# zeehu/generative_ranking_recommender

Measured on AMD Instinct MI355X. Metric: vectors quantized/sec (3-level RQ, 512-d), higher is better.
Workload: dtype f32

## Files before the change

### generative_ranking_recommender_amd/_lib.py

```python
from __future__ import annotations

import contextlib
import ctypes
import fcntl
import os
import subprocess
import tempfile
from pathlib import Path

PKG = Path(__file__).resolve().parent
REPO = PKG.parent
LIB_PATH = PKG / "librqsid.so"
SRCS = [PKG / "csrc" / "rqsid.hip", PKG / "csrc" / "assign.hip", PKG / "csrc" / "assign_stream.hip",
        PKG / "csrc" / "assign_resident.hip", PKG / "csrc" / "assign_rows.hip", PKG / "csrc" / "assign_pc.hip",
        PKG / "csrc" / "auction.hip",
        PKG / "csrc" / "auction_seg.hip", PKG / "csrc" / "quant_error.hip", PKG / "csrc" / "assign_topk.hip",
        PKG / "csrc" / "beam.hip", PKG / "csrc" / "silhouette.hip"]
DEPS = SRCS + [PKG / "csrc" / "internal.h", PKG / "csrc" / "assign_common.h", PKG / "csrc" / "assign_plan.h",
               PKG / "csrc" / "topk_kernel.h", PKG / "csrc" / "exact_row.h"]
HEADER = REPO / "include" / "rqsid.h"
IO_LIB_PATH = PKG / "librqsid_io.so"
IO_SRCS = [PKG / "csrc" / "csv_loader.cpp"]
IO_HEADER = REPO / "include" / "rqsid_io.h"
IO_FLAGS = ["-O3", "-std=c++17", "-Wall", "-shared", "-fPIC", "-pthread"]

HIPCC_FLAGS = ["--offload-arch=gfx950", "-O3", "-std=c++17", "-fno-slp-vectorize", "-shared", "-fPIC"]

c_i32, c_i64, c_f32, c_vp, c_char_p = ctypes.c_int32, ctypes.c_int64, ctypes.c_float, ctypes.c_void_p, ctypes.c_char_p

SIGNATURES = {
    "rqsid_version": (c_i32, []),
    "rqsid_last_error": (c_char_p, []),
    "rqsid_build_flags": (c_i32, []),
    "rqsid_prepare_centers": (c_i32, [c_vp, c_i64, c_i32, c_vp, c_vp, c_vp]),
    "rqsid_prepare_centers_hi": (c_i32, [c_vp, c_i64, c_i32, c_vp, c_vp]),
    "rqsid_bucket_workspace_bytes": (c_i64, [c_i64, c_i32]),
    "rqsid_bucket": (c_i32, [c_vp, c_i64, c_i32, c_i32, c_vp, c_vp, c_vp, c_vp, c_i64, c_vp]),
    "rqsid_assign_tile_rows": (c_i32, []),
    "rqsid_assign_workspace_bytes": (c_i64, [c_i64]),
    "rqsid_assign": (c_i32, [c_vp, c_i64, c_i32, c_vp, c_i32, c_vp, c_vp, c_i64,
                             c_vp, c_vp, c_vp, c_vp, c_i32,
                             c_vp, c_vp, c_i32, c_vp, c_vp, c_vp,
                             c_i32, c_i32, c_vp, c_vp, c_vp, c_vp, c_vp, c_vp,
                             c_vp, c_vp, c_i32, c_vp, c_i64, c_vp]),
    "rqsid_assign_x": (c_i32, [c_vp, c_i32, c_i64, c_i32, c_vp, c_i32, c_vp, c_vp, c_i64,
                               c_vp, c_vp, c_vp, c_vp, c_i32,
                               c_vp, c_vp, c_i32, c_vp, c_vp, c_vp,
                               c_i32, c_i32, c_vp, c_vp, c_vp, c_vp, c_vp, c_vp,
                               c_vp, c_vp, c_i32, c_vp, c_i64, c_vp]),
    "rqsid_pair_table_bytes": (c_i64, [c_i32]),
    "rqsid_pair_table": (c_i32, [c_vp, c_i32, c_vp, c_i32, c_i32, c_vp, c_vp, c_i32, c_vp, c_vp, c_vp]),
    "rqsid_assign_pair": (c_i32, [c_vp, c_i32, c_i64, c_i32, c_vp, c_i32, c_vp, c_vp, c_i64,
                                  c_vp, c_vp, c_vp, c_vp, c_i32,
                                  c_vp, c_vp, c_i32, c_vp, c_vp, c_vp,
                                  c_i32, c_i32, c_vp, c_vp, c_vp, c_vp, c_vp, c_vp,
                                  c_vp, c_vp, c_i32, c_vp, c_i64, c_vp, c_vp]),
    "rqsid_assign_plan_pair": (c_i32, [c_i32, c_i64, c_i32, c_i32, c_i32, c_i32, c_i32, c_i32, c_i32, c_i32, c_i32]),
    "rqsid_assign_topk_workspace_bytes": (c_i64, [c_i64, c_i32]),
    "rqsid_assign_topk": (c_i32, [c_vp, c_i32, c_i64, c_i32, c_vp, c_i32, c_vp, c_vp, c_i64,
                                  c_vp, c_vp, c_i32,
                                  c_vp, c_vp, c_i32, c_vp, c_vp, c_vp,
                                  c_i32, c_i32, c_vp, c_vp, c_vp, c_vp, c_vp, c_vp,
                                  c_i32, c_vp, c_vp, c_vp, c_vp, c_i64, c_vp]),
    "rqsid_beam_expand_workspace_bytes": (c_i64, [c_i64, c_i32]),
    "rqsid_beam_expand": (c_i32, [c_vp, c_i32, c_i64, c_i32, c_i32, c_vp, c_i32, c_vp, c_vp, c_i64,
                                  c_vp, c_vp, c_i32,
                                  c_vp, c_vp, c_i32, c_vp, c_vp, c_vp,
                                  c_i32, c_i32, c_vp, c_vp, c_vp, c_vp, c_vp, c_vp,
                                  c_i32, c_vp, c_vp, c_vp, c_vp, c_i64, c_vp]),
    "rqsid_beam_merge": (c_i32, [c_i64, c_i32, c_i32, c_i32, c_i32, c_vp, c_vp, c_vp, c_vp, c_vp, c_vp,
                                 c_i32, c_i32, c_i32, c_vp, c_vp, c_vp, c_vp, c_vp, c_vp, c_vp]),
    "rqsid_residual": (c_i32, [c_vp, c_i64, c_i32, c_vp, c_i32, c_vp, c_vp, c_i32, c_i32, c_vp, c_vp]),
    "rqsid_quant_error_workspace_bytes": (c_i64, [c_i64]),
    "rqsid_quant_error": (c_i32, [c_vp, c_i32, c_i64, c_i32, c_vp, c_i32, c_i32,
                                  c_vp, c_i32, c_vp, c_vp, c_i32, c_vp, c_vp, c_i32, c_vp,
                                  c_vp, c_vp, c_vp, c_vp, c_i64, c_vp]),
    "rqsid_silhouette_tile_rows": (c_i32, []),
    "rqsid_silhouette_workspace_bytes": (c_i64, [c_i64, c_i32, c_i32]),
    "rqsid_silhouette": (c_i32, [c_vp, c_i32, c_i64, c_i32, c_vp, c_i32, c_vp, c_vp, c_i32, c_vp, c_vp, c_i32,
                                 c_vp, c_vp, c_vp, c_vp, c_vp, c_i64, c_vp]),
    "rqsid_scale_groups": (c_i32, [c_vp, c_i64, c_i32, c_vp, c_i32, c_vp, c_vp, c_vp]),
    "rqsid_centroid_tile_rows": (c_i32, []),
    "rqsid_centroid_accumulate": (c_i32, [c_vp, c_i32, c_vp, c_i32, c_vp, c_vp, c_i64, c_vp, c_vp]),
    "rqsid_centroid_finalize": (c_i32, [c_vp, c_vp, c_i32, c_i32, c_vp, c_vp]),
    "rqsid_match_workspace_bytes": (c_i64, [c_i32]),
    "rqsid_match_to_candidates": (c_i32, [c_vp, c_i32, c_i32, c_vp, c_vp, c_vp, c_vp, c_vp, c_i64, c_vp]),
    "rqsid_pairwise_distance": (c_i32, [c_vp, c_i64, c_i32, c_vp, c_i32, c_vp, c_vp]),
    "rqsid_auction_scores": (c_i32, [c_vp, c_i64, c_i32, c_vp, c_i32, c_i32, c_vp, c_vp]),
    "rqsid_auction_workspace_bytes": (c_i64, [c_i64, c_i32]),
    "rqsid_auction_lap_half": (c_i32, [c_vp, c_i32, c_i64, c_i32, c_vp, c_vp, c_vp, c_i64, c_vp]),
# ... 142 lines not shown
```

### generative_ranking_recommender_amd/csrc/assign.hip

```cpp
#include "assign_common.h"
#include "exact_row.h"

namespace rqsid {
namespace {

__global__ __launch_bounds__(256) void centers_absmax_kernel(const float* __restrict__ c, int64_t n,
                                                             unsigned* __restrict__ out) {
  unsigned m = 0;
  for (int64_t i = (int64_t)blockIdx.x * 256 + threadIdx.x; i < n; i += (int64_t)gridDim.x * 256)
    m = max(m, __float_as_uint(fabsf(c[i])));
  for (int o = 32; o > 0; o >>= 1) m = max(m, (unsigned)__shfl_xor((int)m, o));
  if ((threadIdx.x & 63) == 0) atomicMax(out, m);
}

__global__ __launch_bounds__(256) void prepare_centers_kernel(const float* __restrict__ c, int64_t k, int dim,
                                                              _Float16* __restrict__ c16, float4* __restrict__ meta) {
  const int lane = threadIdx.x & 63;
  const int64_t row = (int64_t)blockIdx.x * 4 + (threadIdx.x >> 6);
  if (row >= k) return;
  const int sx = table_scale_exp(reinterpret_cast<const unsigned*>(meta + k)[0]);
  const float* cr = c + row * dim;
  double s = 0.0, s1 = 0.0, s2 = 0.0;
  for (int i = lane; i < dim; i += 64) {
    const float v = cr[i];
// ... 719 lines not shown
        c8[j + 1] = max(a, bq);
      }
#pragma unroll
    for (int j = 0; j < kMaxList; ++j) w.cand[j] = (uint16_t)(c8[j] == INT_MAX ? 0xFFFF : c8[j]);
    const int n = ncand;
    w.n = n;
  }
  push_work(p, h == 0 && row_valid && !definitive, lane, w);
}

constexpr int screen_min_blocks(int NT, int S, bool T3, int CW) {
  return CW > 1 ? 2 : (T3 ? 2 : (S == 2 ? (NT == 4 ? 3 : 2) : ((NT == 4 && S <= 3) ? 2 : 1)));
}
template <int NT, int S, int RL, bool NORM, bool T3, bool ONE, int CW = 1>
__global__ __launch_bounds__(256 * CW, screen_min_blocks(NT, S, T3, CW)) void assign_screen_kernel(AssignParams p) {
  screen_tile<NT, S, RL, NORM, T3, ONE, CW, RQSID_X_F32>(p);
}
template <int RL, bool NORM>
__global__ __launch_bounds__(256, screen_min_blocks(4, 2, true, 1)) void assign_screen_pair_kernel(AssignParams p) {
  screen_tile<4, 2, RL, NORM, true, true, 1, RQSID_X_F32, true>(p);
}
template <int XF, int NT, int S, int RL, bool NORM, bool T3, bool ONE>
__global__ __launch_bounds__(256, screen_min_blocks(NT, S, T3, 1)) void assign_screen_x16_kernel(AssignParams p) {
  screen_tile<NT, S, RL, NORM, T3, ONE, 1, XF>(p);
}

constexpr int kHalfDim = 512;
static_assert(kHalfDim == kPlanHalfDim, "assign_plan.h constants");

constexpr int kOvfSlot = 56;
template <int RL, bool NORM, int XF, int W>
__device__ __forceinline__ void rescore_rows(const AssignParams& p, const int32_t* __restrict__ ovf_list, int mode) {
  constexpr int G = 64 / W;
  constexpr int kV = (W == 64 ? kMaxDim : kHalfDim) / (4 * W);
  const int lane = threadIdx.x & 63, gl = lane & (W - 1), hh = lane / W;
  const int wid = blockIdx.x * 4 + (threadIdx.x >> 6);
  const int nw = gridDim.x * 4;
  const int64_t nitems_raw = mode == 2 ? p.work_count[kOvfSlot] : *p.work_count;
  const int64_t nitems = nitems_raw < p.work_cap ? nitems_raw : p.work_cap;
  const int nv = p.dim / 4;
  for (int64_t it0 = G * (int64_t)wid; it0 < nitems; it0 += G * (int64_t)nw) {
    const int64_t it = it0 + hh < nitems ? it0 + hh : it0;
    const WorkItem w = p.work[mode == 2 ? ovf_list[it] : (p.work_idx ? p.work_idx[it] : it)];
    const bool active = it0 + hh < nitems && (mode == 0 || (mode == 1 ? w.n != -1 : w.n == -1));
    const float* car = RL >= 1 ? p.ca + (int64_t)seg_row(p.seg_ca, w.seg) * p.dim : nullptr;
    const float* cbr = RL >= 2 ? p.cb + (int64_t)seg_row(p.seg_cb, w.seg) * p.dim : nullptr;
    const bool screened = w.n >= 1 || w.n == -1;
    float4 v[kV];
    const double ss = build_row<RL, NORM, XF, W>(p.x, w.row, p.dim, car, cbr, p.den_in, gl, v);
    if (NORM && RL >= 1) {
      float den;
      if (RL == 1 && p.den_out && screened) den = p.den_out[w.row];
      else den = chain_divisor<W>(ss);
      if (RL == 1 && p.den_out && !screened && gl == 0 && active) p.den_out[w.row] = den;
#pragma unroll
      for (int m = 0; m < kV; ++m) v[m] = div4(v[m], den);
    }
    const bool penalty = w.n == -2;
    const bool listed = w.n >= 1;
    const int base = p.cand_base[w.seg];
    const int n = !active ? 0 : listed ? w.n : (penalty ? p.n_centers : (w.n == -1 ? p.cand_count[w.seg] : 0));
    const int nmax = G == 2 ? max(n, __shfl_xor(n, 32)) : n;
    double best = INFINITY;
    int bj = INT_MAX;
    for (int j0 = 0; j0 < nmax; j0 += kBatch) {
      auto loc = [&](int jj) { return listed ? (int)w.cand[jj] : j0 + jj; };
      double key = batch_dist2<W, double>(v, gl, nv, j0, n, [&](int jj) {
        const int g = penalty ? loc(jj) : cand_global(p, base, loc(jj));
        return reinterpret_cast<const float4*>(p.centers + (int64_t)g * p.dim);
      });
      const int my_jj = batch_slot<W>(gl);
      int my_loc = INT_MAX;
#pragma unroll
      for (int jj = 0; jj < kBatch; ++jj) my_loc = my_jj == jj ? (j0 + jj < n ? loc(jj) : INT_MAX) : my_loc;
      if (penalty) key = (double)((float)sqrt((double)(float)key) + 10000.0f);
      group_min<W>(key, my_loc);
      if (takes(key, my_loc, best, bj)) {
        best = key;
        bj = my_loc;
      }
    }
    if (gl == 0 && active) {
      const bool found = bj != INT_MAX;
      p.out_local[w.row] = found && !penalty ? cand_local(p, base, bj) : -1;
      p.out_global[w.row] = found ? (penalty ? bj : cand_global(p, base, bj)) : -1;
    }
  }
}
template <int RL, bool NORM>
__global__ __launch_bounds__(256) void assign_rescore_kernel(AssignParams p) {
  rescore_rows<RL, NORM, RQSID_X_F32, 64>(p, nullptr, 0);
}
template <int XF, int RL, bool NORM>
__global__ __launch_bounds__(256) void assign_rescore_x16_kernel(AssignParams p) {
  rescore_rows<RL, NORM, XF, 64>(p, nullptr, 0);
}
template <int RL, bool NORM>
__global__ __launch_bounds__(256) void assign_rescore_half_kernel(AssignParams p, const int32_t* __restrict__ ovf_list,
                                                                  int mode) {
  rescore_rows<RL, NORM, RQSID_X_F32, 32>(p, ovf_list, mode);
}
template <int XF, int RL, bool NORM>
__global__ __launch_bounds__(256) void assign_rescore_half_x16_kernel(AssignParams p, const int32_t* __restrict__ ovf_list,
                                                                      int mode) {
  rescore_rows<RL, NORM, XF, 32>(p, ovf_list, mode);
}

__global__ __launch_bounds__(256) void overflow_list_kernel(AssignParams p, int32_t* __restrict__ ovf_list) {
  const int64_t nitems_raw = *p.work_count;
  const int64_t nitems = nitems_raw < p.work_cap ? nitems_raw : p.work_cap;
  for (int64_t it = (int64_t)blockIdx.x * 256 + threadIdx.x; it < nitems; it += (int64_t)gridDim.x * 256) {
    const int32_t idx = p.work_idx ? p.work_idx[it] : (int32_t)it;
    if ((uint32_t)idx >= (uint32_t)p.work_cap) {
      atomicOr(p.work_count + kErrSlot, kErrWorkIdx);
      continue;
    }
    if (p.work[idx].n == -1) {
      const int pos = atomicAdd(p.work_count + kOvfSlot, 1);
      if (pos < p.work_cap) ovf_list[pos] = idx;
      else atomicOr(p.work_count + kErrSlot, kErrOvfList);
    }
  }
}

template <int RL, bool NORM, int XF>
__device__ __forceinline__ void rescreen_rows(const AssignParams& p, const int32_t* __restrict__ ovf_list) {
  constexpr int kV = kHalfDim / 128;
  const int lane = threadIdx.x & 63, hl = lane & 31, hh = lane >> 5;
  const int wid = blockIdx.x * 4 + (threadIdx.x >> 6);
  const int nw = gridDim.x * 4;
  const int64_t nov = p.work_count[kOvfSlot];
  const int nv = p.dim / 4;
  const float eps = (float)(p.dim + 4) * 0x1p-24f * 1.001f;
  for (int64_t it0 = 2 * (int64_t)wid; it0 < nov; it0 += 2 * (int64_t)nw) {
    const bool active = it0 + hh < nov;
    const int32_t idx = ovf_list[active ? it0 + hh : it0];
    WorkItem w = p.work[idx];
    const float* car = RL >= 1 ? p.ca + (int64_t)seg_row(p.seg_ca, w.seg) * p.dim : nullptr;
// ... 277 lines not shown
template <int XF>
void launch_tile_screen(const AssignParams& p, const AssignPlan& plan, int rl, bool norm, unsigned grid, hipStream_t st) {
  if constexpr (XF == RQSID_X_F32) {
    if (plan.pair) {
      const size_t lds = ScreenLayout<4, 2, true>::bytes(rl, p.dim);
      dispatch_rl_norm(rl, norm, [&](auto RL, auto NORM) {
        hipLaunchKernelGGL((assign_screen_pair_kernel<RL(), NORM()>), dim3(grid), dim3(256), lds, st, p);
      });
      return;
    }
    if (plan.cw == 2 && plan.t3) return launch_screen<4, kSplitS, true, true, 2>(p, rl, norm, grid, st);
    if (plan.cw == 2) return launch_screen<8, kSplitS, false, true, 2>(p, rl, norm, grid, st);
  }
  if (plan.t3) launch_screen2<4, 2, true, XF>(p, rl, norm, grid, plan.one, st);
  else if (plan.nt == 4) launch_screen2<4, 2, false, XF>(p, rl, norm, grid, plan.one, st);
  else launch_screen2<8, 2, false, XF>(p, rl, norm, grid, plan.one, st);
}

template <int XF, int RL, bool NORM>
void launch_rescreen(const AssignParams& p, const int32_t* ovf_list, hipStream_t st) {
  if constexpr (XF == RQSID_X_F32)
    hipLaunchKernelGGL((assign_rescreen_kernel<RL, NORM>), dim3(2048), dim3(256), 0, st, p, ovf_list);
  else
    hipLaunchKernelGGL((assign_rescreen_x16_kernel<XF, RL, NORM>), dim3(2048), dim3(256), 0, st, p, ovf_list);
}
template <int XF, int RL, bool NORM>
void launch_rescore_half(const AssignParams& p, const int32_t* ovf_list, int mode, dim3 g, hipStream_t st) {
  if constexpr (XF == RQSID_X_F32)
    hipLaunchKernelGGL((assign_rescore_half_kernel<RL, NORM>), g, dim3(256), 0, st, p, ovf_list, mode);
  else
    hipLaunchKernelGGL((assign_rescore_half_x16_kernel<XF, RL, NORM>), g, dim3(256), 0, st, p, ovf_list, mode);
}
template <int XF, int RL, bool NORM>
void launch_rescore(const AssignParams& p, dim3 g, hipStream_t st) {
  if constexpr (XF == RQSID_X_F32) hipLaunchKernelGGL((assign_rescore_kernel<RL, NORM>), g, dim3(256), 0, st, p);
  else hipLaunchKernelGGL((assign_rescore_x16_kernel<XF, RL, NORM>), g, dim3(256), 0, st, p);
}
template <int XF, int RL, bool NORM>
void launch_exact(const AssignParams& p, const int32_t* ovf_list, bool half, hipStream_t st) {
  const dim3 g(4096);
  if (half && ovf_list) {
    launch_rescore_half<XF, RL, NORM>(p, ovf_list, 1, g, st);
    launch_rescore_half<XF, RL, NORM>(p, ovf_list, 2, g, st);
  } else if (half) {
    launch_rescore_half<XF, RL, NORM>(p, nullptr, 0, g, st);
  } else {
    launch_rescore<XF, RL, NORM>(p, g, st);
  }
}

int env_int(const char* name, int dflt) {
  const char* e = getenv(name);
  return e ? atoi(e) : dflt;
}
AssignEnv read_assign_env() {
  AssignEnv e;
  e.screen_variant = env_int("RQSID_SCREEN_VARIANT", e.screen_variant);
  e.pc = env_int("RQSID_PC", e.pc);
  e.pcw = env_int("RQSID_PCW", e.pcw);
  e.stream_shape = env_int("RQSID_STREAM_SHAPE", e.stream_shape);
  e.rows_shape = env_int("RQSID_ROWS_SHAPE", e.rows_shape);
  e.rescore_full = env_int("RQSID_RESCORE_FULL", e.rescore_full);
  e.no_rescreen = env_int("RQSID_NO_RESCREEN", e.no_rescreen);
  e.no_pair = env_int("RQSID_NO_PAIR", e.no_pair);
  e.test_force_spin_cap = env_int("RQSID_TEST_FORCE_SPIN_CAP", e.test_force_spin_cap);
  return e;
}

}
}

using namespace rqsid;

extern "C" {

int rqsid_prepare_centers(const float* centers, int64_t k, int32_t dim, uint16_t* c16, float* c_meta,
                          void* stream) {
  if (!centers || !c16 || !c_meta || k < 0 || dim <= 0 || dim % kChunk || dim > kMaxDim)
    return fail(RQSID_E_ARG, "prepare_centers: bad arguments (k=%lld dim=%d)", (long long)k, dim);
  if (k == 0) return RQSID_OK;
// ... 127 lines not shown
      break;
    case AssignPlan::kTile:
      if (n_segments > 1) {
        hipLaunchKernelGGL(tile_seg128_kernel, dim3(grid_cap(cdiv(max_tiles, 256), 4096)), dim3(256), 0, st, seg_tile_off,
                           n_segments, n_rows, ws.tile_seg);
        p.tile_seg = ws.tile_seg;
      }
      dispatch_xf(x_format, [&](auto XF) {
        launch_tile_screen<XF()>(p, plan, res_levels, norm, (unsigned)((max_tiles + 7) / 8 * 8), st);
      });
      break;
  }
  if (plan.compact) {
    hipLaunchKernelGGL(sentinel_compact_kernel, dim3((unsigned)cdiv(n_rows, kCompactRows)), dim3(256), 0, st, out_global,
                       n_rows, p.work_count, ws.work_idx, n_rows);
    p.work_idx = ws.work_idx;
  }
  if (plan.expand) launch_resident_expand(p, ws.tile_seg, n_rows, st);
  if ((rc = check_launch("assign_screen"))) return rc;
  const int32_t* ovf_list = nullptr;
  if (plan.rescreen) {
    ovf_list = ws.ovf_list;
    hipLaunchKernelGGL(overflow_list_kernel, dim3(grid_cap(cdiv(n_rows, 256), 1024)), dim3(256), 0, st, p, ws.ovf_list);
    dispatch_xf(x_format, [&](auto XF) {
      constexpr int xf = decltype(XF)::value;
      dispatch_rl_norm(res_levels, norm,
                       [&](auto RL, auto NORM) { launch_rescreen<xf, RL(), NORM()>(p, ovf_list, st); });
    });
    if ((rc = check_launch("assign_rescreen"))) return rc;
  }
  dispatch_xf(x_format, [&](auto XF) {
    constexpr int xf = decltype(XF)::value;
    dispatch_rl_norm(res_levels, norm,
                     [&](auto RL, auto NORM) { launch_exact<xf, RL(), NORM()>(p, ovf_list, plan.half, st); });
  });
  if ((rc = check_launch("assign_rescore"))) return rc;
  if (plan.read_err_word) {
    int32_t err = 0;
    if (hipMemcpyAsync(&err, p.err, 4, hipMemcpyDeviceToHost, st) != hipSuccess || hipStreamSynchronize(st) != hipSuccess)
      return fail(RQSID_E_LAUNCH, "assign: error word readback");
    if (err) return fail(RQSID_E_LAUNCH, "assign: a resident-screen wait reached its spin cap (error word %d)", err);
  }
  return RQSID_OK;
}

int rqsid_assign_x(const void* x, int32_t x_format, int64_t n_rows, int32_t dim, const int32_t* row_index, int32_t n_segments,
                 const int32_t* seg_row_off, const int32_t* seg_tile_off, int64_t max_tiles, const float* centers,
                 const uint16_t* c16, const uint16_t* c16_hi, const float* c_meta, int32_t n_centers,
                 const int32_t* cand_base,
                 const int32_t* cand_count, int32_t cand_count_max, const int32_t* cand_idx,
                 const int32_t* cand_lid, const uint8_t* seg_flags, int32_t res_levels, int32_t res_normalize, const float* ca,
                 const int32_t* seg_ca, const float* cb, const int32_t* seg_cb, const float* den_in,
                 float* den_out, int32_t* out_local, int32_t* out_global, int32_t screen_terms, void* workspace,
                 int64_t workspace_bytes, void* stream) {
  return assign_call(x, x_format, n_rows, dim, row_index, n_segments, seg_row_off, seg_tile_off, max_tiles, centers,
                     c16, c16_hi, c_meta, n_centers, cand_base, cand_count, cand_count_max, cand_idx, cand_lid, seg_flags,
                     res_levels, res_normalize, ca, seg_ca, cb, seg_cb, den_in, den_out, out_local, out_global,
                     screen_terms, workspace, workspace_bytes, stream, nullptr);
}

int rqsid_assign_pair(const void* x, int32_t x_format, int64_t n_rows, int32_t dim, const int32_t* row_index, int32_t n_segments,
                 const int32_t* seg_row_off, const int32_t* seg_tile_off, int64_t max_tiles, const float* centers,
                 const uint16_t* c16, const uint16_t* c16_hi, const float* c_meta, int32_t n_centers,
                 const int32_t* cand_base,
                 const int32_t* cand_count, int32_t cand_count_max, const int32_t* cand_idx,
                 const int32_t* cand_lid, const uint8_t* seg_flags, int32_t res_levels, int32_t res_normalize, const float* ca,
                 const int32_t* seg_ca, const float* cb, const int32_t* seg_cb, const float* den_in,
                 float* den_out, int32_t* out_local, int32_t* out_global, int32_t screen_terms, void* workspace,
                 int64_t workspace_bytes, void* stream, const uint16_t* pair_table) {
  return assign_call(x, x_format, n_rows, dim, row_index, n_segments, seg_row_off, seg_tile_off, max_tiles, centers,
                     c16, c16_hi, c_meta, n_centers, cand_base, cand_count, cand_count_max, cand_idx, cand_lid, seg_flags,
                     res_levels, res_normalize, ca, seg_ca, cb, seg_cb, den_in, den_out, out_local, out_global,
                     screen_terms, workspace, workspace_bytes, stream, pair_table);
}

int32_t rqsid_assign_plan_pair(int32_t x_format, int64_t n_rows, int32_t dim, int32_t n_segments, int32_t cand_count_max,
                               int32_t res_levels, int32_t res_normalize, int32_t screen_terms, int32_t has_cand_lid,
                               int32_t has_den_out, int32_t has_pair) {
  AssignShape shape;
  shape.x_format = x_format;
  shape.n_rows = n_rows;
  shape.dim = dim;
  shape.n_segments = n_segments;
  shape.cand_count_max = cand_count_max;
  shape.res_levels = res_levels;
  shape.norm = res_normalize != 0;
  shape.screen_terms = screen_terms;
  shape.has_cand_lid = has_cand_lid != 0;
  shape.has_den_out = has_den_out != 0;
  shape.has_pair = has_pair != 0;
  return plan_assign(shape, read_assign_env()).pair ? 1 : 0;
}

int64_t rqsid_pair_table_bytes(int32_t n_segments) {
  return (int64_t)(n_segments > 0 ? n_segments : 0) * kPairCand * kPairCand * 2;
}

int rqsid_pair_table(const float* centers, int32_t dim, const float* c_meta, int32_t n_centers, int32_t n_segments,
                     const int32_t* cand_base, const int32_t* cand_count, int32_t cand_count_max, const int32_t* cand_idx,
                     uint16_t* pair_table, void* stream) {
  if (!centers || !c_meta || !cand_base || !cand_count || !pair_table || dim <= 0 || dim % kChunk || dim > kMaxDim ||
      n_centers <= 0 || n_segments <= 0 || n_segments > INT32_MAX / kPairCand || cand_count_max < 0 ||
      cand_count_max > kPairCand || (reinterpret_cast<uintptr_t>(pair_table) & 15))
    return fail(RQSID_E_ARG, "pair_table: bad arguments (dim=%d S=%d K=%d cand_count_max=%d; at most %d candidates per segment)",
                dim, n_segments, n_centers, cand_count_max, kPairCand);
  hipLaunchKernelGGL(pair_table_kernel, dim3((unsigned)n_segments * kPairCand), dim3(256), 0, (hipStream_t)stream, centers,
                     dim, c_meta, n_centers, cand_base, cand_count, cand_idx, reinterpret_cast<_Float16*>(pair_table));
  return check_launch("pair_table");
}

int rqsid_assign(const float* x, int64_t n_rows, int32_t dim, const int32_t* row_index, int32_t n_segments,
                 const int32_t* seg_row_off, const int32_t* seg_tile_off, int64_t max_tiles, const float* centers,
                 const uint16_t* c16, const uint16_t* c16_hi, const float* c_meta, int32_t n_centers,
                 const int32_t* cand_base,
                 const int32_t* cand_count, int32_t cand_count_max, const int32_t* cand_idx,
                 const int32_t* cand_lid, const uint8_t* seg_flags, int32_t res_levels, int32_t res_normalize, const float* ca,
                 const int32_t* seg_ca, const float* cb, const int32_t* seg_cb, const float* den_in,
                 float* den_out, int32_t* out_local, int32_t* out_global, int32_t screen_terms, void* workspace,
                 int64_t workspace_bytes, void* stream) {
  return rqsid_assign_x(x, RQSID_X_F32, n_rows, dim, row_index, n_segments, seg_row_off, seg_tile_off, max_tiles, centers,
                        c16, c16_hi, c_meta, n_centers, cand_base, cand_count, cand_count_max, cand_idx, cand_lid, seg_flags,
                        res_levels, res_normalize, ca, seg_ca, cb, seg_cb, den_in, den_out, out_local, out_global,
                        screen_terms, workspace, workspace_bytes, stream);
}

#ifdef RQSID_STAMPS
// ... 19 lines not shown
```

### generative_ranking_recommender_amd/csrc/assign_plan.h

```cpp
#pragma once
#include <cstdint>

namespace rqsid {

constexpr int kPlanXF32 = 0;
constexpr int kPlanMaxList = 8;
constexpr int kPlanSplitDim = 512;
constexpr int kPlanHalfDim = 512;
constexpr int kPlanStreamDim = 512;
constexpr int kPlanStreamMinRows = 64 * 256;
constexpr int kPlanPcDim = 512;
constexpr int kPlanPcRows = 128;
constexpr int kPlanPcDescBytes = 32;
constexpr int kPlanResDim = 512;
constexpr int kPlanRowsDim = 512;
constexpr int kPlanRowsMaxCand = 512;
constexpr int kPlanPairCand = 128;
constexpr int kPlanWorkItemBytes = 32;
constexpr int kPlanDescBytesPerRow = 16;

struct AssignWorkspaceMap {
  int64_t header = 0, work = 256, tile_seg, work_idx, desc, ovf_list, total_bytes;
  explicit AssignWorkspaceMap(int64_t n_rows) {
    const int64_t n = n_rows > 0 ? n_rows : 0, ints = (n * 4 + 255) / 256 * 256;
// ... 22 lines not shown
  bool has_cand_lid = false;
  bool has_den_out = false;
  bool has_pair = false;
};

struct AssignEnv {
  int screen_variant = 0;
  int pc = 1;
  int pcw = 0;
  int stream_shape = 83;
  int rows_shape = 443;
  int rescore_full = 0;
  int no_rescreen = 0;
  int no_pair = 0;
  int test_force_spin_cap = 0;
};

struct AssignPlan {
  enum Screen { kTile, kStream, kRows, kResident, kPc };
  Screen screen = kTile;
  bool t3 = false;
  bool pair = false;
  int nt = 4;
  bool one = false;
  int cw = 1;
  int s = 2;
  int stream_shape = 0;
  int rows_shape = 0;
  bool pc_wide = false;
  bool compact = false;
  bool expand = false;
  bool rescreen = false;
  bool half = false;
  bool force_cap = false;
  bool read_err_word = false;
};

inline bool stream_supported(int nt, bool t3, int rl) {
  if (nt == 8) return !t3 && rl >= 0 && rl <= 2;
  if (nt == 4) return rl >= 0 && rl <= 2;
  return false;
}
inline bool rows_supported(int dim, int cand_count_max, bool t3, int rl, bool norm) {
  return dim == kPlanRowsDim && !t3 && cand_count_max > 0 && cand_count_max <= kPlanRowsMaxCand && rl >= 0 && rl <= 2 &&
         !(rl == 1 && norm);
}
inline bool resident_supported(int dim, int cand_count_max, bool t3) {
  return dim == kPlanResDim && cand_count_max >= 1 && cand_count_max <= 256 && !t3;
}
inline bool pc_supported(int dim, int cand_count_max, bool t3, int rl) {
  if (dim != kPlanPcDim || rl < 1 || rl > 2) return false;
  return t3 ? cand_count_max <= 128 : cand_count_max <= 256;
}
inline int64_t pc_desc_bytes(int64_t n_rows, int32_t n_segments) {
  return ((n_rows > 0 ? n_rows : 0) / kPlanPcRows + (int64_t)n_segments + 1) * kPlanPcDescBytes;
}

inline AssignPlan plan_assign(const AssignShape& a, const AssignEnv& e) {
  AssignPlan pl;
  const int ccm = a.cand_count_max, rl = a.res_levels, variant = e.screen_variant;
  const bool x16 = a.x_format != kPlanXF32;
  const bool want3 = a.screen_terms == 3 || a.screen_terms == 2;
  const bool t3 = (ccm <= 128 && (want3 || (a.screen_terms == 0 && rl >= 1))) ||
                  (ccm <= 256 && (want3 || (a.screen_terms == 0 && rl == 1)));
  const bool legacy = variant == 2;
  pl.t3 = t3;
  pl.nt = t3 || ccm <= 128 ? 4 : 8;
  pl.half = a.dim <= kPlanHalfDim && !e.rescore_full;
  pl.rescreen = a.dim <= kPlanHalfDim && !e.no_rescreen && ccm > kPlanMaxList;

  const bool persistent_ok =
      !x16 && (int64_t)a.n_segments + 1 <= a.n_rows && (rl != 1 || !a.norm || a.has_den_out);
  const bool want_pc = variant == 9 || (variant == 0 && (e.pc >= 2 || (e.pc == 1 && !t3)));
  const bool want_rows = variant == 8 || (variant == 0 && rl >= 1 && ccm > 256);
  const int want_stream = variant == 5 ? (e.stream_shape == 42 || e.stream_shape == 88 ? e.stream_shape : 83)
                                       : (variant == 0 && pl.nt == 8 && !t3 && rl >= 1 ? 88 : 0);
  if (persistent_ok && want_pc && pc_supported(a.dim, ccm, t3, rl) &&
      pc_desc_bytes(a.n_rows, a.n_segments) <= a.n_rows * kPlanDescBytesPerRow) {
    pl.screen = AssignPlan::kPc;
    pl.nt = t3 ? 4 : 8;
    pl.pc_wide = !t3 && e.pcw == 1;
    pl.compact = true;
  } else if (persistent_ok && want_rows && rows_supported(a.dim, ccm, t3, rl, a.norm)) {
    pl.screen = AssignPlan::kRows;
    pl.rows_shape = e.rows_shape == 482 || e.rows_shape == 883 ? e.rows_shape : 443;
  } else if (persistent_ok && variant == 6 && resident_supported(a.dim, ccm, t3)) {
    pl.screen = AssignPlan::kResident;
    pl.compact = pl.expand = pl.read_err_word = true;
    pl.force_cap = e.test_force_spin_cap != 0;
  } else if (persistent_ok && want_stream && a.dim == kPlanStreamDim && ccm <= 256 && !a.has_cand_lid &&
             a.n_rows >= kPlanStreamMinRows && stream_supported(pl.nt, t3, rl)) {
    pl.screen = AssignPlan::kStream;
    pl.stream_shape = want_stream;
    pl.compact = true;
  } else {
    const bool split = !x16 && !legacy && variant != 7 && a.dim <= kPlanSplitDim;
    const int one_pass = pl.nt * 32;
    if (ccm <= one_pass) {
      pl.one = !legacy;
      pl.pair = t3 && pl.one && !x16 && a.has_pair && !e.no_pair && a.screen_terms != 3;
    } else if (ccm <= 2 * one_pass && split) {
// ... 10 lines not shown
```

### generative_ranking_recommender_amd/csrc/exact_row.h

```cpp
#pragma once
#include <type_traits>

#include "assign_common.h"

namespace rqsid {

constexpr int kBatch = 8;

__device__ __forceinline__ float4 sub4(float4 a, float4 c) {
  return make_float4(a.x - c.x, a.y - c.y, a.z - c.z, a.w - c.w);
}
__device__ __forceinline__ float4 div4(float4 a, float d) { return make_float4(a.x / d, a.y / d, a.z / d, a.w / d); }
__device__ __forceinline__ double sq4(float4 a) {
  return (double)a.x * a.x + (double)a.y * a.y + (double)a.z * a.z + (double)a.w * a.w;
}

__device__ __forceinline__ float4 chain4(float4 a, int rl, bool norm, float4 ca, float4 cb, float den_in) {
  if (rl >= 1) a = sub4(a, ca);
  if (rl >= 2) {
    if (norm) a = div4(a, den_in);
    a = sub4(a, cb);
  }
  return a;
}
__device__ __forceinline__ float4 chain4(float4 a, int rl, bool norm, float4 ca, float4 cb, float den_in, float den) {
  a = chain4(a, rl, norm, ca, cb, den_in);
  if (norm && rl >= 1) a = div4(a, den);
  return a;
}

template <int W>
__device__ __forceinline__ double group_sum(double v) {
#pragma unroll
  for (int o = W / 2; o > 0; o >>= 1) v += __shfl_xor(v, o);
  return v;
}
template <int W>
__device__ __forceinline__ float chain_divisor(double ss) {
  return (float)sqrt(group_sum<W>(ss)) + 1e-8f;
}

template <int RL, bool NORM, int XF, int W, int MV>
__device__ __forceinline__ double build_row(const float* x, int64_t row, int dim, const float* car, const float* cbr,
                                            const float* den_in, int gl, float4 (&v)[MV]) {
  const int nv = dim / 4;
  const float4 z4 = make_float4(0.f, 0.f, 0.f, 0.f);
  double ss = 0.0;
#pragma unroll
  for (int m = 0; m < MV; ++m) {
    const int i = gl + W * m;
    if (i < nv) {
      const float4 ca = RL >= 1 ? reinterpret_cast<const float4*>(car)[i] : z4;
      const float4 cb = RL >= 2 ? reinterpret_cast<const float4*>(cbr)[i] : z4;
      const float d1 = (RL >= 2 && NORM) ? den_in[row] : 1.0f;
      const float4 a = chain4(load_row4<XF>(x, row, dim, i), RL, NORM, ca, cb, d1);
      v[m] = a;
      ss += sq4(a);
    } else {
      v[m] = z4;
    }
  }
  return ss;
}

template <int W, typename T, int MV>
__device__ __forceinline__ T cand_dist2(const float4 (&v)[MV], const float4* cr, int gl, int nv) {
  T acc = 0;
#pragma unroll
  for (int m = 0; m < MV; ++m) {
    const int i = gl + W * m;
    if (i < nv) {
      const float4 c = cr[i];
      if constexpr (std::is_same_v<T, double>) {
        const double d0 = (double)v[m].x - c.x, d1 = (double)v[m].y - c.y, d2 = (double)v[m].z - c.z,
                     d3 = (double)v[m].w - c.w;
        acc += d0 * d0 + d1 * d1 + d2 * d2 + d3 * d3;
      } else {
        const float d0 = v[m].x - c.x, d1 = v[m].y - c.y, d2 = v[m].z - c.z, d3 = v[m].w - c.w;
        acc = fmaf(d0, d0, fmaf(d1, d1, fmaf(d2, d2, fmaf(d3, d3, acc))));
      }
    }
  }
  return acc;
}

template <int W>
__device__ __forceinline__ int batch_slot(int gl) {
  constexpr int s = __builtin_ctz(W / 8);
  return 4 * ((gl >> (s + 2)) & 1) + 2 * ((gl >> (s + 1)) & 1) + ((gl >> s) & 1);
}
template <int W>
__device__ __forceinline__ constexpr int batch_lane(int jj) {
  return (W / 2) * ((jj >> 2) & 1) + (W / 4) * ((jj >> 1) & 1) + (W / 8) * (jj & 1);
}
template <int W, typename T>
__device__ __forceinline__ T batch_reduce(const T (&acc)[kBatch], int gl) {
  T r4[4], r2[2], r1;
  const bool hi = gl & (W / 2), mid = gl & (W / 4), lo = gl & (W / 8);
#pragma unroll
  for (int j = 0; j < 4; ++j) r4[j] = (hi ? acc[j + 4] : acc[j]) + __shfl_xor(hi ? acc[j] : acc[j + 4], W / 2);
#pragma unroll
  for (int j = 0; j < 2; ++j) r2[j] = (mid ? r4[j + 2] : r4[j]) + __shfl_xor(mid ? r4[j] : r4[j + 2], W / 4);
  r1 = (lo ? r2[1] : r2[0]) + __shfl_xor(lo ? r2[0] : r2[1], W / 8);
#pragma unroll
  for (int o = W / 16; o > 0; o >>= 1) r1 += __shfl_xor(r1, o);
  return r1;
}
template <int W, typename T, int MV, typename F>
__device__ __forceinline__ T batch_dist2(const float4 (&v)[MV], int gl, int nv, int j0, int n, F&& row) {
  T acc[kBatch];
#pragma unroll
  for (int jj = 0; jj < kBatch; ++jj) {
    acc[jj] = 0;
    if (j0 + jj < n) acc[jj] = cand_dist2<W, T>(v, row(jj), gl, nv);
  }
  return batch_reduce<W>(acc, gl);
}

__device__ __forceinline__ bool takes(double ok, int ol, double key, int loc) {
  const bool kn = key != key, okn = ok != ok;
  return ol != INT_MAX && (loc == INT_MAX || (!okn && (kn || ok < key || (ok == key && ol < loc))));
}
template <int W>
__device__ __forceinline__ void group_min(double& key, int& loc) {
#pragma unroll
  for (int o = W / 8; o < W; o <<= 1) {
    const double ok = __shfl_xor(key, o);
    const int ol = __shfl_xor(loc, o);
    const bool take = takes(ok, ol, key, loc);
    key = take ? ok : key;
    loc = take ? ol : loc;
  }
}

}
```

### include/rqsid.h

```cpp
#ifndef RQSID_H
#define RQSID_H
#include <stdint.h>

#ifdef __cplusplus
extern "C" {
#endif

#define RQSID_OK 0
#define RQSID_E_ARG (-1)
#define RQSID_E_LAUNCH (-2)
#define RQSID_E_WORKSPACE (-3)

#define RQSID_SEG_PENALTY 1u

#define RQSID_X_F32 0
#define RQSID_X_F16 1
#define RQSID_X_BF16 2

int rqsid_version(void);
const char* rqsid_last_error(void);
int32_t rqsid_build_flags(void);

int rqsid_prepare_centers(const float* centers, int64_t k, int32_t dim,
                          uint16_t* c16, float* c_meta, void* stream);
// ... 21 lines not shown
                 void* workspace, int64_t workspace_bytes, void* stream);
int rqsid_assign_x(const void* x, int32_t x_format, int64_t n_rows, int32_t dim, const int32_t* row_index,
                   int32_t n_segments, const int32_t* seg_row_off, const int32_t* seg_tile_off,
                   int64_t max_tiles,
                   const float* centers, const uint16_t* c16, const uint16_t* c16_hi, const float* c_meta,
                   int32_t n_centers,
                   const int32_t* cand_base, const int32_t* cand_count, int32_t cand_count_max,
                   const int32_t* cand_idx, const int32_t* cand_lid, const uint8_t* seg_flags,
                   int32_t res_levels, int32_t res_normalize,
                   const float* ca, const int32_t* seg_ca, const float* cb, const int32_t* seg_cb,
                   const float* den_in, float* den_out,
                   int32_t* out_local, int32_t* out_global, int32_t screen_terms,
                   void* workspace, int64_t workspace_bytes, void* stream);

int64_t rqsid_pair_table_bytes(int32_t n_segments);
int rqsid_pair_table(const float* centers, int32_t dim, const float* c_meta, int32_t n_centers, int32_t n_segments,
                     const int32_t* cand_base, const int32_t* cand_count, int32_t cand_count_max,
                     const int32_t* cand_idx, uint16_t* pair_table, void* stream);
int rqsid_assign_pair(const void* x, int32_t x_format, int64_t n_rows, int32_t dim, const int32_t* row_index,
                      int32_t n_segments, const int32_t* seg_row_off, const int32_t* seg_tile_off,
                      int64_t max_tiles,
                      const float* centers, const uint16_t* c16, const uint16_t* c16_hi, const float* c_meta,
                      int32_t n_centers,
                      const int32_t* cand_base, const int32_t* cand_count, int32_t cand_count_max,
                      const int32_t* cand_idx, const int32_t* cand_lid, const uint8_t* seg_flags,
                      int32_t res_levels, int32_t res_normalize,
                      const float* ca, const int32_t* seg_ca, const float* cb, const int32_t* seg_cb,
                      const float* den_in, float* den_out,
                      int32_t* out_local, int32_t* out_global, int32_t screen_terms,
                      void* workspace, int64_t workspace_bytes, void* stream, const uint16_t* pair_table);
int32_t rqsid_assign_plan_pair(int32_t x_format, int64_t n_rows, int32_t dim, int32_t n_segments,
                               int32_t cand_count_max, int32_t res_levels, int32_t res_normalize,
                               int32_t screen_terms, int32_t has_cand_lid, int32_t has_den_out, int32_t has_pair);

#define RQSID_TOPK_MAX 8
int64_t rqsid_assign_topk_workspace_bytes(int64_t n_rows, int32_t k);
int rqsid_assign_topk(const void* x, int32_t x_format, int64_t n_rows, int32_t dim, const int32_t* row_index,
                      int32_t n_segments, const int32_t* seg_row_off, const int32_t* seg_tile_off, int64_t max_tiles,
                      const float* centers, const float* c_meta, int32_t n_centers,
                      const int32_t* cand_base, const int32_t* cand_count, int32_t cand_count_max,
                      const int32_t* cand_idx, const int32_t* cand_lid, const uint8_t* seg_flags,
                      int32_t res_levels, int32_t res_normalize,
                      const float* ca, const int32_t* seg_ca, const float* cb, const int32_t* seg_cb,
                      const float* den_in, float* den_out,
                      int32_t k, int32_t* out_local, int32_t* out_global, float* out_dist,
                      void* workspace, int64_t workspace_bytes, void* stream);

int64_t rqsid_beam_expand_workspace_bytes(int64_t n_items, int32_t k);
int rqsid_beam_expand(const void* x, int32_t x_format, int64_t n_items, int32_t beam, int32_t dim,
                      const int32_t* row_index,
                      int32_t n_segments, const int32_t* seg_row_off, const int32_t* seg_tile_off, int64_t max_tiles,
                      const float* centers, const float* c_meta, int32_t n_centers,
                      const int32_t* cand_base, const int32_t* cand_count, int32_t cand_count_max,
                      const int32_t* cand_idx, const int32_t* cand_lid, const uint8_t* seg_flags,
                      int32_t res_levels, int32_t res_normalize,
                      const float* ca, const int32_t* seg_ca, const float* cb, const int32_t* seg_cb,
                      const float* den_in, float* den_out,
                      int32_t k, int32_t* out_local, int32_t* out_global, float* out_dist,
                      void* workspace, int64_t workspace_bytes, void* stream);

int rqsid_beam_merge(int64_t n_rows, int32_t beam_in, int32_t k, int32_t beam_out, int32_t level,
                     const int32_t* exp_local, const int32_t* exp_global, const float* exp_dist,
                     const float* scale_in, const float* den, const int32_t* path_in,
                     int32_t use_global, int32_t key_mult, int32_t dead_key,
                     int32_t* path_out, float* scale_out, float* den_next, float* rec_out,
                     int32_t* key_out, int32_t* src_out, void* stream);
// ... 107 lines not shown
```

Before: 630.8 million.

## Add quarter-wave (16-lane) exact rescore path with split partial accumulators

Adds a rescore variant where each row is handled by 16 lanes instead of 32, so four rows are processed per wave, and makes it the default for dim <= 512. Each lane keeps two partial accumulators per candidate and the batch size per pass is halved, which changes the shuffle reduction tree and the candidate indexing. The goal is to raise row-level parallelism and cut idle lanes in the overflow rescore pass. The cost is more registers per lane, a launch bound that requests higher occupancy, and more batch iterations per row.

```diff
diff --git a/generative_ranking_recommender_amd/_lib.py b/generative_ranking_recommender_amd/_lib.py
--- a/generative_ranking_recommender_amd/_lib.py
+++ b/generative_ranking_recommender_amd/_lib.py
@@ -56,6 +56,7 @@
                                   c_i32, c_i32, c_vp, c_vp, c_vp, c_vp, c_vp, c_vp,
                                   c_vp, c_vp, c_i32, c_vp, c_i64, c_vp, c_vp]),
     "rqsid_assign_plan_pair": (c_i32, [c_i32, c_i64, c_i32, c_i32, c_i32, c_i32, c_i32, c_i32, c_i32, c_i32, c_i32]),
+    "rqsid_assign_plan_rescore_lanes": (c_i32, [c_i32, c_i32]),
     "rqsid_assign_topk_workspace_bytes": (c_i64, [c_i64, c_i32]),
     "rqsid_assign_topk": (c_i32, [c_vp, c_i32, c_i64, c_i32, c_vp, c_i32, c_vp, c_vp, c_i64,
                                   c_vp, c_vp, c_i32,
diff --git a/generative_ranking_recommender_amd/csrc/assign.hip b/generative_ranking_recommender_amd/csrc/assign.hip
--- a/generative_ranking_recommender_amd/csrc/assign.hip
+++ b/generative_ranking_recommender_amd/csrc/assign.hip
@@ -775,6 +775,8 @@
 template <int RL, bool NORM, int XF, int W>
 __device__ __forceinline__ void rescore_rows(const AssignParams& p, const int32_t* __restrict__ ovf_list, int mode) {
   constexpr int G = 64 / W;
+  constexpr int P = W == 16 ? 2 : 1;
+  constexpr int kB = kBatch / P;
   constexpr int kV = (W == 64 ? kMaxDim : kHalfDim) / (4 * W);
   const int lane = threadIdx.x & 63, gl = lane & (W - 1), hh = lane / W;
   const int wid = blockIdx.x * 4 + (threadIdx.x >> 6);
@@ -790,11 +792,12 @@
     const float* cbr = RL >= 2 ? p.cb + (int64_t)seg_row(p.seg_cb, w.seg) * p.dim : nullptr;
     const bool screened = w.n >= 1 || w.n == -1;
     float4 v[kV];
-    const double ss = build_row<RL, NORM, XF, W>(p.x, w.row, p.dim, car, cbr, p.den_in, gl, v);
+    double ss[P];
+    build_row<RL, NORM, XF, W, P>(p.x, w.row, p.dim, car, cbr, p.den_in, gl, v, ss);
     if (NORM && RL >= 1) {
       float den;
       if (RL == 1 && p.den_out && screened) den = p.den_out[w.row];
-      else den = chain_divisor<W>(ss);
+      else den = chain_divisor<W, P>(ss);
       if (RL == 1 && p.den_out && !screened && gl == 0 && active) p.den_out[w.row] = den;
 #pragma unroll
       for (int m = 0; m < kV; ++m) v[m] = div4(v[m], den);
@@ -803,21 +806,26 @@
     const bool listed = w.n >= 1;
     const int base = p.cand_base[w.seg];
     const int n = !active ? 0 : listed ? w.n : (penalty ? p.n_centers : (w.n == -1 ? p.cand_count[w.seg] : 0));
-    const int nmax = G == 2 ? max(n, __shfl_xor(n, 32)) : n;
+    int nmax = n;
+#pragma unroll
+    for (int o = W; o < 64; o <<= 1) nmax = max(nmax, __shfl_xor(nmax, o));
+    nmax = __builtin_amdgcn_readfirstlane(nmax);
     double best = INFINITY;
     int bj = INT_MAX;
-    for (int j0 = 0; j0 < nmax; j0 += kBatch) {
-      auto loc = [&](int jj) { return listed ? (int)w.cand[jj] : j0 + jj; };
-      double key = batch_dist2<W, double>(v, gl, nv, j0, n, [&](int jj) {
+    for (int j0 = 0; j0 < nmax; j0 += kB) {
+      auto loc = [&](int jj) {
+        return !listed ? j0 + jj : (int)(kB < kMaxList && j0 ? w.cand[(jj + kB) % kMaxList] : w.cand[jj]);
+      };
+      double key = batch_dist2<W, double, P>(v, gl, nv, j0, n, P == 2 ? nmax - j0 : kB, [&](int jj) {
         const int g = penalty ? loc(jj) : cand_global(p, base, loc(jj));
         return reinterpret_cast<const float4*>(p.centers + (int64_t)g * p.dim);
       });
-      const int my_jj = batch_slot<W>(gl);
+      const int my_jj = batch_slot<W * P>(gl);
       int my_loc = INT_MAX;
 #pragma unroll
-      for (int jj = 0; jj < kBatch; ++jj) my_loc = my_jj == jj ? (j0 + jj < n ? loc(jj) : INT_MAX) : my_loc;
+      for (int jj = 0; jj < kB; ++jj) my_loc = my_jj == jj ? (j0 + jj < n ? loc(jj) : INT_MAX) : my_loc;
       if (penalty) key = (double)((float)sqrt((double)(float)key) + 10000.0f);
-      group_min<W>(key, my_loc);
+      group_min<W, P>(key, my_loc);
       if (takes(key, my_loc, best, bj)) {
         best = key;
         bj = my_loc;
@@ -847,6 +855,17 @@
 __global__ __launch_bounds__(256) void assign_rescore_half_x16_kernel(AssignParams p, const int32_t* __restrict__ ovf_list,
                                                                       int mode) {
   rescore_rows<RL, NORM, XF, 32>(p, ovf_list, mode);
+}
+constexpr int kQuarterWaves = 4;
+template <int RL, bool NORM>
+__global__ __launch_bounds__(256, kQuarterWaves) void assign_rescore_quarter_kernel(AssignParams p, const int32_t* __restrict__ ovf_list,
+                                                                     int mode) {
+  rescore_rows<RL, NORM, RQSID_X_F32, 16>(p, ovf_list, mode);
+}
+template <int XF, int RL, bool NORM>
+__global__ __launch_bounds__(256, kQuarterWaves) void assign_rescore_quarter_x16_kernel(AssignParams p,
+                                                                         const int32_t* __restrict__ ovf_list, int mode) {
+  rescore_rows<RL, NORM, XF, 16>(p, ovf_list, mode);
 }
 
 __global__ __launch_bounds__(256) void overflow_list_kernel(AssignParams p, int32_t* __restrict__ ovf_list) {
@@ -1190,20 +1209,30 @@
     hipLaunchKernelGGL((assign_rescore_half_x16_kernel<XF, RL, NORM>), g, dim3(256), 0, st, p, ovf_list, mode);
 }
 template <int XF, int RL, bool NORM>
+void launch_rescore_quarter(const AssignParams& p, const int32_t* ovf_list, int mode, dim3 g, hipStream_t st) {
+  if constexpr (XF == RQSID_X_F32)
+    hipLaunchKernelGGL((assign_rescore_quarter_kernel<RL, NORM>), g, dim3(256), 0, st, p, ovf_list, mode);
+  else
+    hipLaunchKernelGGL((assign_rescore_quarter_x16_kernel<XF, RL, NORM>), g, dim3(256), 0, st, p, ovf_list, mode);
+}
+template <int XF, int RL, bool NORM>
 void launch_rescore(const AssignParams& p, dim3 g, hipStream_t st) {
   if constexpr (XF == RQSID_X_F32) hipLaunchKernelGGL((assign_rescore_kernel<RL, NORM>), g, dim3(256), 0, st, p);
   else hipLaunchKernelGGL((assign_rescore_x16_kernel<XF, RL, NORM>), g, dim3(256), 0, st, p);
 }
 template <int XF, int RL, bool NORM>
-void launch_exact(const AssignParams& p, const int32_t* ovf_list, bool half, hipStream_t st) {
+void launch_exact(const AssignParams& p, const int32_t* ovf_list, int lanes, hipStream_t st) {
   const dim3 g(4096);
-  if (half && ovf_list) {
-    launch_rescore_half<XF, RL, NORM>(p, ovf_list, 1, g, st);
-    launch_rescore_half<XF, RL, NORM>(p, ovf_list, 2, g, st);
-  } else if (half) {
-    launch_rescore_half<XF, RL, NORM>(p, nullptr, 0, g, st);
+  if (lanes == 64) return launch_rescore<XF, RL, NORM>(p, g, st);
+  const auto pass = [&](int mode) {
+    if (lanes == 16) launch_rescore_quarter<XF, RL, NORM>(p, ovf_list, mode, g, st);
+    else launch_rescore_half<XF, RL, NORM>(p, ovf_list, mode, g, st);
+  };
+  if (ovf_list) {
+    pass(1);
+    pass(2);
   } else {
-    launch_rescore<XF, RL, NORM>(p, g, st);
+    pass(0);
   }
 }
 
@@ -1397,7 +1426,7 @@
   dispatch_xf(x_format, [&](auto XF) {
     constexpr int xf = decltype(XF)::value;
     dispatch_rl_norm(res_levels, norm,
-                     [&](auto RL, auto NORM) { launch_exact<xf, RL(), NORM()>(p, ovf_list, plan.half, st); });
+                     [&](auto RL, auto NORM) { launch_exact<xf, RL(), NORM()>(p, ovf_list, plan.rescore_lanes, st); });
   });
   if ((rc = check_launch("assign_rescore"))) return rc;
   if (plan.read_err_word) {
@@ -1457,6 +1486,13 @@
   return plan_assign(shape, read_assign_env()).pair ? 1 : 0;
 }
 
+int32_t rqsid_assign_plan_rescore_lanes(int32_t x_format, int32_t dim) {
+  AssignShape shape;
+  shape.x_format = x_format;
+  shape.dim = dim;
+  return plan_assign(shape, read_assign_env()).rescore_lanes;
+}
+
 int64_t rqsid_pair_table_bytes(int32_t n_segments) {
   return (int64_t)(n_segments > 0 ? n_segments : 0) * kPairCand * kPairCand * 2;
 }
diff --git a/generative_ranking_recommender_amd/csrc/assign_plan.h b/generative_ranking_recommender_amd/csrc/assign_plan.h
--- a/generative_ranking_recommender_amd/csrc/assign_plan.h
+++ b/generative_ranking_recommender_amd/csrc/assign_plan.h
@@ -78,6 +78,7 @@
   bool expand = false;
   bool rescreen = false;
   bool half = false;
+  int rescore_lanes = 64;
   bool force_cap = false;
   bool read_err_word = false;
 };
@@ -112,7 +113,8 @@
   const bool legacy = variant == 2;
   pl.t3 = t3;
   pl.nt = t3 || ccm <= 128 ? 4 : 8;
-  pl.half = a.dim <= kPlanHalfDim && !e.rescore_full;
+  pl.half = a.dim <= kPlanHalfDim && e.rescore_full != 1;
+  pl.rescore_lanes = !pl.half ? 64 : (e.rescore_full == 2 ? 32 : 16);
   pl.rescreen = a.dim <= kPlanHalfDim && !e.no_rescreen && ccm > kPlanMaxList;
 
   const bool persistent_ok =
diff --git a/generative_ranking_recommender_amd/csrc/exact_row.h b/generative_ranking_recommender_amd/csrc/exact_row.h
--- a/generative_ranking_recommender_amd/csrc/exact_row.h
+++ b/generative_ranking_recommender_amd/csrc/exact_row.h
@@ -35,17 +35,27 @@
   for (int o = W / 2; o > 0; o >>= 1) v += __shfl_xor(v, o);
   return v;
 }
+template <int W, int P>
+__device__ __forceinline__ double group_sum(const double (&v)[P]) {
+  static_assert(P == 1 || P == 2, "one partial per lane, or two");
+  return group_sum<W>(P == 2 ? v[0] + v[P - 1] : v[0]);
+}
 template <int W>
 __device__ __forceinline__ float chain_divisor(double ss) {
   return (float)sqrt(group_sum<W>(ss)) + 1e-8f;
 }
+template <int W, int P>
+__device__ __forceinline__ float chain_divisor(const double (&ss)[P]) {
+  return (float)sqrt(group_sum<W, P>(ss)) + 1e-8f;
+}
 
-template <int RL, bool NORM, int XF, int W, int MV>
-__device__ __forceinline__ double build_row(const float* x, int64_t row, int dim, const float* car, const float* cbr,
-                                            const float* den_in, int gl, float4 (&v)[MV]) {
+template <int RL, bool NORM, int XF, int W, int P, int MV>
+__device__ __forceinline__ void build_row(const float* x, int64_t row, int dim, const float* car, const float* cbr,
+                                          const float* den_in, int gl, float4 (&v)[MV], double (&ss)[P]) {
   const int nv = dim / 4;
   const float4 z4 = make_float4(0.f, 0.f, 0.f, 0.f);
-  double ss = 0.0;
+#pragma unroll
+  for (int p = 0; p < P; ++p) ss[p] = 0.0;
 #pragma unroll
   for (int m = 0; m < MV; ++m) {
     const int i = gl + W * m;
@@ -55,17 +65,24 @@
       const float d1 = (RL >= 2 && NORM) ? den_in[row] : 1.0f;
       const float4 a = chain4(load_row4<XF>(x, row, dim, i), RL, NORM, ca, cb, d1);
       v[m] = a;
-      ss += sq4(a);
+      ss[m % P] += sq4(a);
     } else {
       v[m] = z4;
     }
   }
-  return ss;
+}
+template <int RL, bool NORM, int XF, int W, int MV>
+__device__ __forceinline__ double build_row(const float* x, int64_t row, int dim, const float* car, const float* cbr,
+                                            const float* den_in, int gl, float4 (&v)[MV]) {
+  double ss[1];
+  build_row<RL, NORM, XF, W, 1>(x, row, dim, car, cbr, den_in, gl, v, ss);
+  return ss[0];
 }
 
-template <int W, typename T, int MV>
-__device__ __forceinline__ T cand_dist2(const float4 (&v)[MV], const float4* cr, int gl, int nv) {
-  T acc = 0;
+template <int W, typename T, int P, int MV>
+__device__ __forceinline__ void cand_dist2(const float4 (&v)[MV], const float4* cr, int gl, int nv, T (&acc)[P]) {
+#pragma unroll
+  for (int p = 0; p < P; ++p) acc[p] = 0;
 #pragma unroll
   for (int m = 0; m < MV; ++m) {
     const int i = gl + W * m;
@@ -74,14 +91,13 @@
       if constexpr (std::is_same_v<T, double>) {
         const double d0 = (double)v[m].x - c.x, d1 = (double)v[m].y - c.y, d2 = (double)v[m].z - c.z,
                      d3 = (double)v[m].w - c.w;
-        acc += d0 * d0 + d1 * d1 + d2 * d2 + d3 * d3;
+        acc[m % P] += d0 * d0 + d1 * d1 + d2 * d2 + d3 * d3;
       } else {
         const float d0 = v[m].x - c.x, d1 = v[m].y - c.y, d2 = v[m].z - c.z, d3 = v[m].w - c.w;
-        acc = fmaf(d0, d0, fmaf(d1, d1, fmaf(d2, d2, fmaf(d3, d3, acc))));
+        acc[m % P] = fmaf(d0, d0, fmaf(d1, d1, fmaf(d2, d2, fmaf(d3, d3, acc[m % P]))));
       }
     }
   }
-  return acc;
 }
 
 template <int W>
@@ -93,38 +109,59 @@
 __device__ __forceinline__ constexpr int batch_lane(int jj) {
   return (W / 2) * ((jj >> 2) & 1) + (W / 4) * ((jj >> 1) & 1) + (W / 8) * (jj & 1);
 }
-template <int W, typename T>
-__device__ __forceinline__ T batch_reduce(const T (&acc)[kBatch], int gl) {
-  T r4[4], r2[2], r1;
-  const bool hi = gl & (W / 2), mid = gl & (W / 4), lo = gl & (W / 8);
+template <int S, typename T>
+__device__ __forceinline__ T reduce4(const T (&r4)[4], int gl) {
+  T r2[2], r1;
+  const bool mid = gl & S, lo = gl & (S / 2);
 #pragma unroll
-  for (int j = 0; j < 4; ++j) r4[j] = (hi ? acc[j + 4] : acc[j]) + __shfl_xor(hi ? acc[j] : acc[j + 4], W / 2);
+  for (int j = 0; j < 2; ++j) r2[j] = (mid ? r4[j + 2] : r4[j]) + __shfl_xor(mid ? r4[j] : r4[j + 2], S);
+  r1 = (lo ? r2[1] : r2[0]) + __shfl_xor(lo ? r2[0] : r2[1], S / 2);
 #pragma unroll
-  for (int j = 0; j < 2; ++j) r2[j] = (mid ? r4[j + 2] : r4[j]) + __shfl_xor(mid ? r4[j] : r4[j + 2], W / 4);
-  r1 = (lo ? r2[1] : r2[0]) + __shfl_xor(lo ? r2[0] : r2[1], W / 8);
+  for (int o = S / 4; o > 0; o >>= 1) r1 += __shfl_xor(r1, o);
+  return r1;
+}
+template <int W, typename T, int P>
+__device__ __forceinline__ T batch_reduce(const T (&acc)[kBatch / P][P], int gl) {
+  static_assert(P == 1 || P == 2, "one partial per lane, or two");
+  T r4[4];
+  if constexpr (P == 1) {
+    const bool hi = gl & (W / 2);
 #pragma unroll
-  for (int o = W / 16; o > 0; o >>= 1) r1 += __shfl_xor(r1, o);
-  return r1;
+    for (int j = 0; j < 4; ++j)
+      r4[j] = (hi ? acc[j + 4][0] : acc[j][0]) + __shfl_xor(hi ? acc[j][0] : acc[j + 4][0], W / 2);
+  } else {
+#pragma unroll
+    for (int j = 0; j < 4; ++j) r4[j] = acc[j][0] + acc[j][P - 1];
+  }
+  return reduce4<W * P / 4>(r4, gl);
+}
+template <int W, typename T, int P, int MV, typename F>
+__device__ __forceinline__ T batch_dist2(const float4 (&v)[MV], int gl, int nv, int j0, int n, int nb, F&& row) {
+  T acc[kBatch / P][P];
+#pragma unroll
+  for (int jj = 0; jj < kBatch / P; ++jj)
+#pragma unroll
+    for (int p = 0; p < P; ++p) acc[jj][p] = 0;
+#pragma unroll
+  for (int jj = 0; jj < kBatch / P; ++jj) {
+    if (jj >= nb) break;
+    if (j0 + jj < n) cand_dist2<W, T, P>(v, row(jj), gl, nv, acc[jj]);
+  }
+  return batch_reduce<W, T, P>(acc, gl);
 }
 template <int W, typename T, int MV, typename F>
 __device__ __forceinline__ T batch_dist2(const float4 (&v)[MV], int gl, int nv, int j0, int n, F&& row) {
-  T acc[kBatch];
-#pragma unroll
-  for (int jj = 0; jj < kBatch; ++jj) {
-    acc[jj] = 0;
-    if (j0 + jj < n) acc[jj] = cand_dist2<W, T>(v, row(jj), gl, nv);
-  }
-  return batch_reduce<W>(acc, gl);
+  return batch_dist2<W, T, 1>(v, gl, nv, j0, n, kBatch, row);
 }
 
 __device__ __forceinline__ bool takes(double ok, int ol, double key, int loc) {
   const bool kn = key != key, okn = ok != ok;
   return ol != INT_MAX && (loc == INT_MAX || (!okn && (kn || ok < key || (ok == key && ol < loc))));
 }
-template <int W>
+template <int W, int P = 1>
 __device__ __forceinline__ void group_min(double& key, int& loc) {
 #pragma unroll
-  for (int o = W / 8; o < W; o <<= 1) {
+  for (int o = W * P / 8; o < W; o <<= 1) {
     const double ok = __shfl_xor(key, o);
     const int ol = __shfl_xor(loc, o);
     const bool take = takes(ok, ol, key, loc);
diff --git a/include/rqsid.h b/include/rqsid.h
--- a/include/rqsid.h
+++ b/include/rqsid.h
@@ -77,6 +77,7 @@
 int32_t rqsid_assign_plan_pair(int32_t x_format, int64_t n_rows, int32_t dim, int32_t n_segments,
                                int32_t cand_count_max, int32_t res_levels, int32_t res_normalize,
                                int32_t screen_terms, int32_t has_cand_lid, int32_t has_den_out, int32_t has_pair);
+int32_t rqsid_assign_plan_rescore_lanes(int32_t x_format, int32_t dim);
 
 #define RQSID_TOPK_MAX 8
 int64_t rqsid_assign_topk_workspace_bytes(int64_t n_rows, int32_t k);
```

After: 633.7 million (median of 6 runs). About the same (+0.5%).
